# ParaGroup/WindFlow

Hardware: AMD Instinct MI355X
Metric: tuples_per_sec (higher is better)
Workload: dtype bf16; 1 GPU; model=keyed_ffat_cb_window, global_batch=16777216, win=1000, slide=100, keys_per_rank=8192, parallelism=keyed-dp1, dense_keys=True

## Files before the change

csrc/engine/bindings.cpp:

```cpp
#include <pybind11/functional.h>
#include <pybind11/numpy.h>
#include <pybind11/pybind11.h>
#include <pybind11/stl.h>

#include "engine.hpp"

namespace py = pybind11;
using namespace wfa;

static py::array col_view(DType dt, void* data, int64_t n) {
    switch (dt) {
        case DType::I64: return py::array_t<int64_t>({n}, {8}, (int64_t*)data, py::none());
        case DType::F64: return py::array_t<double>({n}, {8}, (double*)data, py::none());
        case DType::F32: return py::array_t<float>({n}, {4}, (float*)data, py::none());
        case DType::U64: return py::array_t<uint64_t>({n}, {8}, (uint64_t*)data, py::none());
        case DType::I32: return py::array_t<int32_t>({n}, {4}, (int32_t*)data, py::none());
        case DType::U16: return py::array_t<uint16_t>({n}, {2}, (uint16_t*)data, py::none());
        case DType::U8: return py::array_t<uint8_t>({n}, {1}, (uint8_t*)data, py::none());
    }
    throw std::runtime_error("bad dtype");
}

static py::dict batch_views(Batch* b, RuntimeCtx* ctx = nullptr) {
    py::dict d;
// ... 507 lines not shown
                     e.start();
                     e.wait();
                 }
             })
        .def("start",
             [](Engine& e) {
                 e.build();
                 e.start();
             })
        .def("start_gated",
             [](Engine& e) {
                 e.build();
                 {
                     py::gil_scoped_release rel;
                     e.start_gated();
                 }
             })
        .def("open_gate_and_wait",
             [](Engine& e) {
                 py::gil_scoped_release rel;
                 e.open_gate();
                 e.wait();
             })
        .def("wait",
             [](Engine& e) {
                 py::gil_scoped_release rel;
                 e.wait();
             })
        .def("abort_now", [](Engine& e) { e.abort.store(true); })
        .def("sink_sum", [](Engine& e, int op) { return e.sink_acc_i64.at(op).load(); })
        .def("sink_sum_f",
             [](Engine& e, int op) {
                 std::lock_guard<std::mutex> g(e.sink_f64_mu);
                 auto it = e.sink_acc_f64.find(op);
                 return it == e.sink_acc_f64.end() ? 0.0 : it->second;
             })
        .def("sink_count", [](Engine& e, int op) { return e.sink_tuples.at(op).load(); })
        .def("dropped", [](Engine& e) { return e.dropped_tuples.load(); })
        .def("sink_latencies",
             [](Engine& e, int op) {
                 auto it = e.sink_latencies.find(op);
                 return it == e.sink_latencies.end() ? std::vector<int64_t>{}
                                                     : it->second;
             })
        .def("stats", [](Engine& e) {
            py::list out;
            for (auto& r : e.replicas) {
                py::dict d;
                d["op"] = r->op_id;
                d["name"] = e.ops[r->op_id].name;
                d["replica"] = r->idx;
                d["inputs"] = r->stats.inputs_received;
                d["tuples_in"] = r->stats.tuples_received;
                d["outputs"] = r->stats.outputs_sent;
                d["tuples_out"] = r->stats.tuples_sent;
                d["svc_us_ewma"] = r->stats.service_time_us_ewma;
                d["start_us"] = r->stats.start_us;
                d["end_us"] = r->stats.end_us;
                d["kernels"] = r->stats.num_kernels;
                d["bytes_h2d"] = r->stats.bytes_h2d;
                d["bytes_d2h"] = r->stats.bytes_d2h;
                out.append(d);
            }
            return out;
        });

    m.def("hash_key", [](uint64_t k) { return KeyByEmitter::mix(k); });

#ifdef WFA_WITH_HIP
    m.def("debug_jit_fold_source",
          [](const std::string& kind, const std::string& spec,
             const std::vector<double>& fp, const std::vector<int64_t>& ip) {
              return debug_jit_fold_source(kind, spec, fp, ip);
          });
    m.def("debug_sort_pairs",
          [](py::array_t<uint32_t> keys, int bits) {
              auto r = debug_sort_pairs_host(keys.data(), keys.shape(0), bits);
              py::array_t<uint32_t> ks((py::ssize_t)r.first.size());
              py::array_t<uint32_t> vs((py::ssize_t)r.second.size());
              memcpy(ks.mutable_data(), r.first.data(), 4 * r.first.size());
              memcpy(vs.mutable_data(), r.second.data(), 4 * r.second.size());
              return py::make_tuple(ks, vs);
          });
    m.def("debug_ffat_stage_times",
          [](int64_t n, int64_t n_keys, int64_t win, int64_t slide, int iters,
             int vik, const std::string& fold_variant) {
              py::dict d;
              for (auto& [k, v] : debug_ffat_stage_times(n, n_keys, win, slide,
                                                         iters, vik, fold_variant))
                  d[py::str(k)] = v;
              return d;
          },
          py::arg("n"), py::arg("n_keys"), py::arg("win") = 1000,
          py::arg("slide") = 100, py::arg("iters") = 20, py::arg("vik") = 0,
          py::arg("fold_variant") = "");
    m.def("debug_tb_stage_times",
          [](int64_t n, int64_t n_keys, int iters, int mono) {
              std::map<std::string, double> m2;
              for (auto& kv : debug_tb_stage_times(n, n_keys, iters, mono))
                  m2[kv.first] = kv.second;
              return m2;
          },
          py::arg("n"), py::arg("n_keys"), py::arg("iters") = 20,
          py::arg("mono") = 1);
    m.def("debug_gram_stage_times",
          [](int64_t n, int64_t n_keys, int64_t win, int iters) {
              std::map<std::string, double> m2;
              for (auto& kv : debug_gram_stage_times(n, n_keys, win, iters))
                  m2[kv.first] = kv.second;
              return m2;
          },
          py::arg("n"), py::arg("n_keys"), py::arg("win") = 32,
          py::arg("iters") = 20);
    m.def("debug_a2a_stage_times",
          [](int64_t n, int64_t n_keys, int iters) {
              py::list out;
              for (auto& [k, v] : debug_a2a_stage_times(n, n_keys, iters))
                  out.append(py::make_tuple(k, v));
              return out;
          },
          py::arg("n"), py::arg("n_keys") = 8192, py::arg("iters") = 20);
    m.def("debug_key_slots",
          [](py::array_t<uint64_t> keys, int64_t max_keys) {
              auto r = debug_key_slots_host(keys.data(), keys.shape(0), max_keys);
              py::array_t<uint32_t> s((py::ssize_t)r.size());
              memcpy(s.mutable_data(), r.data(), 4 * r.size());
              return s;
          });
#endif

    struct StateStore {
        std::shared_ptr<void> holder;
        void* kv = nullptr;
        void* cache = nullptr;
    };
    py::class_<StateStore>(m, "StateStore")
        .def(py::init([](const std::string& path, int64_t cache_cap, bool fresh) {
                 auto s = new StateStore();
                 s->holder =
                     open_state_store(path, cache_cap, &s->kv, &s->cache, fresh);
                 return s;
             }),
             py::arg("path"), py::arg("cache_capacity") = 1 << 16,
             py::arg("fresh") = true)
        .def("erase",
             [](StateStore& s, uint64_t key) {
                 return state_kv_erase(s.kv, s.cache, key);
             })
        .def("get",
             [](StateStore& s, uint64_t key) -> py::object {
                 std::string* v = state_cache_get(s.cache, key);
                 if (!v) return py::none();
                 return py::bytes(*v);
             })
        .def("put",
             [](StateStore& s, uint64_t key, py::bytes val) {
                 state_cache_put(s.cache, key, std::string(val));
             })
        .def("flush", [](StateStore& s) { state_cache_flush(s.cache); })
        .def("__len__", [](StateStore& s) { return state_kv_size(s.kv); });
}
```

csrc/engine/engine.hpp:

```cpp
#pragma once

#include <chrono>
#include <deque>
#include <functional>
#include <thread>
#include <unordered_map>

#include "core.hpp"
#include "queue.hpp"

namespace wfa {

struct Engine;
struct Replica;

inline int64_t now_us() {
    return std::chrono::duration_cast<std::chrono::microseconds>(
               std::chrono::steady_clock::now().time_since_epoch())
        .count();
}

struct StatsRecord {
    int64_t inputs_received = 0;
    int64_t tuples_received = 0;
// ... 309 lines not shown
    std::atomic<int> gate{0};
    std::atomic<int> warmed{0};
    bool use_gate = false;
    std::unordered_map<int, std::atomic<int64_t>> sink_acc_i64;
    std::unordered_map<int, double> sink_acc_f64;
    std::mutex sink_f64_mu;
    std::unordered_map<int, std::atomic<int64_t>> sink_tuples;
    std::unordered_map<int, std::vector<int64_t>> sink_latencies;
    int64_t queue_capacity = 128;
    bool pin_threads = false;
    int dist_rank = 0;
    int dist_world = 1;
    std::string rccl_id;

    Pool* make_pool(const Schema& s, int64_t cap, bool pinned) {
        pools.push_back(std::make_unique<Pool>(s, cap, pinned));
        return pools.back().get();
    }

    void build();
    void start();
    void wait();
    void run() { build(); start(); wait(); }
    void start_gated();
    void open_gate() { gate.store(1, std::memory_order_release); }
};

std::shared_ptr<OpLogic> make_native_logic(const std::string& kind,
                                           const std::string& spec,
                                           const std::vector<double>& fparams,
                                           const std::vector<int64_t>& iparams,
                                           Engine* eng, int op_id);

struct WinRows {
    int64_t n = 0;
    const int64_t* ts = nullptr;
    uint64_t key = 0;
    int64_t gwid = 0;
    const Schema* schema = nullptr;
    std::vector<const char*> cols;
};
using WindowFn = std::function<double(const WinRows&)>;

struct JoinPairs {
    int64_t n = 0;
    const uint64_t* key = nullptr;
    const int64_t* ts_a = nullptr;
    const int64_t* ts_b = nullptr;
    const double* va = nullptr;
    const double* vb = nullptr;
};
using JoinFn =
    std::function<void(const JoinPairs&, uint8_t* keep, double* out)>;

std::shared_ptr<OpLogic> make_window_logic(const std::string& kind,
                                           const std::vector<double>& fp,
                                           const std::vector<int64_t>& ip,
                                           Engine* eng, int op_id,
                                           WindowFn userfn = nullptr,
                                           JoinFn joinfn = nullptr);

std::shared_ptr<OpLogic> make_gpu_logic(const std::string& kind, const std::string& spec,
                                        const std::vector<double>& fp,
                                        const std::vector<int64_t>& ip, Engine* eng,
                                        int op_id, int device, const Schema& os,
                                        int64_t out_batch);

std::shared_ptr<OpLogic> make_persist_logic(const std::string& kind,
                                            const std::string& spec,
                                            const std::vector<double>& fp,
                                            const std::vector<int64_t>& ip,
                                            Engine* eng, int op_id);
std::shared_ptr<void> open_state_store(const std::string& path, int64_t cache_cap,
                                       void** kv_out, void** cache_out,
                                       bool fresh = true);
std::string* state_cache_get(void* cache, uint64_t key);
void state_cache_put(void* cache, uint64_t key, const std::string& v);
void state_cache_flush(void* cache);
int64_t state_kv_size(void* kv);
bool state_kv_erase(void* kv, void* cache, uint64_t key);

std::pair<std::vector<uint32_t>, std::vector<uint32_t>> debug_sort_pairs_host(
    const uint32_t* keys, int64_t n, int bits);
std::vector<uint32_t> debug_key_slots_host(const uint64_t* keys, int64_t n,
                                           int64_t max_keys);
std::vector<std::pair<std::string, double>> debug_ffat_stage_times(
    int64_t n, int64_t n_keys, int64_t win, int64_t slide, int iters, int vik,
    const std::string& fold_variant = "");
std::vector<std::pair<std::string, double>> debug_gram_stage_times(
    int64_t n, int64_t n_keys, int64_t win, int iters);
std::vector<std::pair<std::string, double>> debug_tb_stage_times(
    int64_t n, int64_t n_keys, int iters, int mono);
std::vector<std::pair<std::string, double>> debug_a2a_stage_times(
    int64_t n, int64_t n_keys, int iters);

std::string wfa_rccl_unique_id();

std::string debug_jit_fold_source(const std::string& kind,
                                  const std::string& spec,
                                  const std::vector<double>& fp,
                                  const std::vector<int64_t>& ip);

}
```

csrc/engine/gpu_ops.cpp:

```cpp
#include <cstring>
#include <deque>
#include <map>
#include <tuple>

#include "engine.hpp"

#ifdef WFA_WITH_HIP
#include <rccl/rccl.h>

#include "../hip/wfa_kernels.h"
#include "gpu_common.hpp"

namespace wfa {

struct AuxPool {
    std::mutex mu;
    std::vector<std::pair<void*, int64_t*>> free_list;
    std::pair<void*, int64_t*> get(int device) {
        {
            std::lock_guard<std::mutex> g(mu);
            if (!free_list.empty()) {
                auto p = free_list.back();
                free_list.pop_back();
                return p;
// ... 1413 lines not shown
        hipEvent_t ev_free = ev_dest[dest_flip];
        dest_flip ^= 1;
        if (db->ready_event)
            HIPCHK(hipStreamWaitEvent(meta_stream, (hipEvent_t)db->ready_event, 0));
        HIPCHK(hipStreamWaitEvent(meta_stream, ev_free, 0));
        wfa_bucket_by_key_h(meta_stream, db->key, n, world, dest, hi);
        wfa_count_u32(meta_stream, dest, n, d_counts, world);
        HIPCHK(hipEventRecord(ev_counts, meta_stream));
        start_meta(true, wm, false);
        Meta m = sync_meta(true);
        if (m.remote_in == 0 && m.remote_out == 0 &&
            !getenv("WFA_XCHG_NO_SELFPASS")) {
            release(sb);
            int64_t out_wm = m.min_wm == WM_MAX ? cur_wm : m.min_wm;
            cur_wm = std::max(cur_wm, out_wm);
            db->watermark = out_wm;
            if (ctx.stats) ctx.stats->num_kernels += 3;
            out.emit(db);
            if (wfa_prof())
                fprintf(stderr, "[prof] xchg n=%ld self-forward meta=%ld us\n",
                        (long)n, (long)(now_us() - t1));
            return;
        }
        HIPCHK(hipStreamWaitEvent(stream, ev_counts, 0));
        uint32_t *od, *oi;
        wfa_sort_pairs2_ph(stream, dest, idx, dest_t, idx_t, nullptr, nullptr,
                           hi, n, bits, &od, &oi, nullptr, 1,
                           0);
        HIPCHK(hipEventRecord(ev_free, stream));
        size_t nc = db->cols.size();
        std::vector<void*> ptrs(2 * nc);
        for (size_t c = 0; c < nc; ++c) {
            ptrs[c] = db->cols[c];
            ptrs[nc + c] = sb->cols[c];
        }
        HIPCHK(hipMemcpyAsync(d_colptrs, ptrs.data(), 8 * 2 * nc,
                              hipMemcpyHostToDevice, stream));
        wfa_gather_rows(stream, oi, n, db->ts, sb->ts, db->key, sb->key,
                        (const void* const*)d_colptrs, (void* const*)(d_colptrs + nc),
                        d_esize, (int)nc);
        release_after_use(db);
        if (ctx.stats) ctx.stats->num_kernels += 4;
        int64_t t2 = now_us();
        round(sb, out, ctx);
        release(sb);
        if (wfa_prof())
            fprintf(stderr, "[prof] xchg n=%ld in+get=%ld us bucket=%ld us round=%ld us\n",
                    (long)n, (long)(t1 - t0), (long)(t2 - t1), (long)(now_us() - t2));
    }

    bool on_punct(int64_t, EmitCtx&, RuntimeCtx&) override { return true; }

    void on_eos(EmitCtx& out, RuntimeCtx& ctx) override {
        ensure_init();
        if (world == 1 && !getenv("WFA_XCHG_NO_SELFPASS")) return;
        for (;;) {
            start_meta(false, cur_wm, true);
            if (round(nullptr, out, ctx)) break;
        }
    }
};

std::pair<std::vector<uint32_t>, std::vector<uint32_t>> debug_sort_pairs_host(
    const uint32_t* keys, int64_t n, int bits) {
    HIPCHK(hipSetDevice(0));
    auto& A = arena(0);
    uint32_t* d_k = (uint32_t*)A.get(4 * n);
    uint32_t* d_v = (uint32_t*)A.get(4 * n);
    uint32_t* d_kt = (uint32_t*)A.get(4 * n);
    uint32_t* d_vt = (uint32_t*)A.get(4 * n);
    uint32_t* d_h = (uint32_t*)A.get(4 * wfa_sort_hist_u32(n));
    HIPCHK(hipMemcpy(d_k, keys, 4 * n, hipMemcpyHostToDevice));
    wfa_iota_u32(nullptr, d_v, n);
    uint32_t *ok, *ov;
    wfa_sort_pairs(nullptr, d_k, d_v, d_kt, d_vt, d_h, n, bits, &ok, &ov);
    std::vector<uint32_t> hk(n), hv(n);
    HIPCHK(hipMemcpy(hk.data(), ok, 4 * n, hipMemcpyDeviceToHost));
    HIPCHK(hipMemcpy(hv.data(), ov, 4 * n, hipMemcpyDeviceToHost));
    A.put(d_k, 4 * n); A.put(d_v, 4 * n); A.put(d_kt, 4 * n); A.put(d_vt, 4 * n);
    A.put(d_h, 4 * wfa_sort_hist_u32(n));
    return {std::move(hk), std::move(hv)};
}

std::vector<uint32_t> debug_key_slots_host(const uint64_t* keys, int64_t n,
                                           int64_t max_keys) {
    HIPCHK(hipSetDevice(0));
    auto& A = arena(0);
    int64_t cap = 1;
    while (cap < 2 * max_keys) cap <<= 1;
    uint64_t* d_key = (uint64_t*)A.get(8 * n);
    uint64_t* d_tab = (uint64_t*)A.get(16 * cap);
    uint32_t* d_ns = (uint32_t*)A.get(64);
    uint32_t* d_out = (uint32_t*)A.get(4 * n);
    uint64_t* d_s2k = (uint64_t*)A.get(8 * max_keys);
    HIPCHK(hipMemcpy(d_key, keys, 8 * n, hipMemcpyHostToDevice));
    wfa_fill_u64(nullptr, d_tab, ~0ULL, 2 * cap);
    wfa_fill_u32(nullptr, d_ns, 0, 1);
    wfa_key_to_slot(nullptr, d_key, n, d_tab, d_ns, cap, d_out, d_s2k);
    std::vector<uint32_t> out(n);
    HIPCHK(hipMemcpy(out.data(), d_out, 4 * n, hipMemcpyDeviceToHost));
    A.put(d_key, 8 * n); A.put(d_tab, 16 * cap);
    A.put(d_ns, 64); A.put(d_out, 4 * n); A.put(d_s2k, 8 * max_keys);
    return out;
}

std::shared_ptr<OpLogic> make_gpu_logic(const std::string& kind, const std::string& spec,
                                        const std::vector<double>& fp,
                                        const std::vector<int64_t>& ip, Engine* eng,
                                        int op_id, int device, const Schema& os,
                                        int64_t out_batch) {
    if (kind == "gpu_source")
        return std::make_shared<GpuSourceLogic>(ip[0], ip[1], ip[2], (int)ip[3],
                                                (uint64_t)ip[4], device, os);
    if (kind == "gpu_map")
        return std::make_shared<GpuMapLogic>((int)ip[0], (int)ip[1], fp[0], fp[1],
                                             device, os);
    if (kind == "gpu_filter")
        return std::make_shared<GpuFilterLogic>((int)ip[0], (int)ip[1], fp[0], fp[1],
                                                device, os, out_batch);
    if (kind == "gpu_jit_map")
        return std::make_shared<GpuJitMapLogic>(spec, (int)(ip.empty() ? 0 : ip[0]),
                                                device, os);
    if (kind == "gpu_jit_filter")
        return std::make_shared<GpuJitFilterLogic>(spec, (int)(ip.empty() ? 0 : ip[0]),
                                                   device, os, out_batch);
    if (kind == "gpu_jit_reduce" || kind == "gpu_jit_ffat" ||
        kind == "gpu_jit_stateful" || kind == "gpu_split")
        return make_gpu_jit_logic(kind, spec, fp, ip, eng, op_id, device, os,
                                  out_batch);
    if (kind == "gpu_map_keyed")
        return std::make_shared<GpuStatefulMapLogic>((int)ip[0], (int)ip[1], fp[0],
                                                     fp[1], ip[2], device, os,
                                                     out_batch);
    if (kind == "gpu_filter_keyed")
        return std::make_shared<GpuStatefulFilterLogic>((int)ip[0], (int)ip[1], fp[0],
                                                        fp[1], ip[2], device, os,
                                                        out_batch);
    if (kind == "gpu_reduce_all")
        return std::make_shared<GpuReduceAllLogic>((int)ip[0], (int)ip[1], device,
                                                   os, out_batch);
    if (kind == "gpu_reduce")
        return std::make_shared<GpuReduceLogic>((int)ip[0], (int)ip[1], ip[2], device,
                                                os, out_batch,
                                                ip.size() > 3 && ip[3] != 0);
    if (kind == "gpu_ffat") {
        auto l = std::make_shared<GpuFfatLogic>(
            (int)ip[0], (int)ip[1], ip[2], ip[3], ip[4], ip[5] != 0, device, os,
            out_batch, ip.size() > 6 && ip[6] != 0, ip.size() > 7 ? ip[7] : 0,
            ip.size() > 8 ? (int)ip[8] : 0, ip.size() > 9 && ip[9] != 0);
        l->eng_ = eng;
        return l;
    }
    if (kind == "gpu_gram") {
        auto l = std::make_shared<GpuGramLogic>(ip[0], ip[1], device, os,
                                                out_batch);
        l->ks.dense = ip.size() > 2 && ip[2] != 0;
        return l;
    }
    if (kind == "gpu_exchange")
        return std::make_shared<GpuExchangeLogic>(eng, device, os, out_batch);
    if (kind == "gpu_to_host")
        return std::make_shared<GpuToHostLogic>(device);
    if (kind == "gpu_count_sink") {
        eng->sink_acc_i64[op_id].store(0);
        eng->sink_tuples[op_id].store(0);
        return std::make_shared<GpuCountSink>(eng, op_id, device);
// ... 298 lines not shown
    float* d_cols[16];
    for (int c = 0; c < 16; ++c) {
        d_cols[c] = (float*)A.get(4 * n);
        wfa_gen_batch(s, d_ts, d_key, d_cols[c], 2, n, 0, 1000 + c, n_keys);
    }
    int64_t fires16 = (n / std::max<int64_t>(win, 1) + n_keys + 64) * 16;
    uint32_t* st_fill = (uint32_t*)A.get(4 * n_keys);
    uint32_t* st_head = (uint32_t*)A.get(4 * n_keys);
    float* st_acc = (float*)A.get(4 * n_keys * 256);
    uint32_t* nf = (uint32_t*)A.get(4 * (fires16 + 1));
    uint64_t* o_key = (uint64_t*)A.get(8 * fires16);
    int64_t* o_gwid = (int64_t*)A.get(8 * fires16);
    int64_t* o_ts = (int64_t*)A.get(8 * fires16);
    float* o_cols[16];
    for (int c = 0; c < 16; ++c) o_cols[c] = (float*)A.get(4 * fires16);
    int64_t* d_on = (int64_t*)A.get(64);
    uint32_t* d_inv = (uint32_t*)A.get(4 * n);
    float* d_staged = (float*)A.get(64 * n);
    const float** d_in = (const float**)A.get(16 * 8);
    float** d_out = (float**)A.get(16 * 8);
    HIPCHK(hipMemcpyAsync(d_in, d_cols, 16 * 8, hipMemcpyHostToDevice, s));
    HIPCHK(hipMemcpyAsync(d_out, o_cols, 16 * 8, hipMemcpyHostToDevice, s));
    HIPCHK(hipMemsetAsync(st_fill, 0, 4 * n_keys, s));
    HIPCHK(hipMemsetAsync(st_head, 0, 4 * n_keys, s));
    HIPCHK(hipMemsetAsync(st_acc, 0, 4 * n_keys * 256, s));

    constexpr int NS = 5;
    const char* names[NS] = {"group", "fire_offsets", "stage_rows", "mfma_fold",
                             "gflops"};
    hipEvent_t ev[NS];
    for (auto& e : ev) HIPCHK(hipEventCreate(&e));
    double acc[NS] = {0};
    RuntimeCtx rctx;
    for (int it = -2; it < iters; ++it) {
        HIPCHK(hipEventRecord(ev[0], s));
        wfa_key_to_slot(s, d_key, n, ks.tab, ks.d_nslots, ks.table_cap,
                        ks.slot, ks.slot_to_key);
        uint32_t *os_, *oi;
        wfa_sort_pairs2(s, ks.slot, ks.idx, ks.slot_t, ks.idx_t, nullptr,
                        nullptr, ks.hist, n, ks.bits, &os_, &oi, nullptr, 1, 0);
        ks.segs(s, os_, n, 0);
        HIPCHK(hipEventRecord(ev[1], s));
        wfa_ffat_fire_offsets(s, ks.seg_start, ks.seg_slot, ks.d_nseg, n, win,
                              1, 1, st_fill, st_head, nf, d_on, nullptr,
                              nullptr, nullptr);
        HIPCHK(hipEventRecord(ev[2], s));
        wfa_gram_prep(s, d_in, oi, n, d_inv, d_staged);
        HIPCHK(hipEventRecord(ev[3], s));
        wfa_gram_fold(s, ks.seg_start, ks.seg_slot, ks.d_nseg, n, d_in, oi,
                      d_ts, win, st_fill, st_acc, st_head, ks.slot_to_key, nf,
                      o_key, o_gwid, d_out, o_ts, fires16, d_on, d_inv,
                      d_staged);
        HIPCHK(hipEventRecord(ev[4], s));
        HIPCHK(hipStreamSynchronize(s));
        if (it >= 0)
            for (int k = 0; k < NS - 1; ++k) {
                float ms = 0;
                HIPCHK(hipEventElapsedTime(&ms, ev[k], ev[k + 1]));
                acc[k] += ms * 1000.0;
            }
    }
    for (auto& e : ev) (void)hipEventDestroy(e);
    std::vector<std::pair<std::string, double>> out;
    for (int k = 0; k < NS - 1; ++k) out.push_back({names[k], acc[k] / iters});
    double fold_us = acc[3] / iters;
    out.push_back({"gflops", fold_us > 0 ? (512.0 * n) / (fold_us * 1e3) : 0});
    return out;
}

}

#else

namespace wfa {
Batch* gpu_alloc_batch(Pool&) { throw std::runtime_error("built without HIP"); }
void gpu_free_batch(Batch*) {}
void gpu_resolve_count(Batch*) {}
Batch* gpu_clone_batch(Batch*) { throw std::runtime_error("built without HIP"); }
std::string wfa_rccl_unique_id() { throw std::runtime_error("built without HIP"); }
std::pair<std::vector<uint32_t>, std::vector<uint32_t>> debug_sort_pairs_host(
    const uint32_t*, int64_t, int) {
    throw std::runtime_error("built without HIP");
}
std::vector<uint32_t> debug_key_slots_host(const uint64_t*, int64_t, int64_t) {
    throw std::runtime_error("built without HIP");
}
std::vector<std::pair<std::string, double>> debug_ffat_stage_times(int64_t, int64_t,
                                                                   int64_t, int64_t,
                                                                   int, int,
                                                                   const std::string&) {
    throw std::runtime_error("built without HIP");
}
std::vector<std::pair<std::string, double>> debug_a2a_stage_times(int64_t, int64_t,
                                                                  int) {
    throw std::runtime_error("built without HIP");
}
std::vector<std::pair<std::string, double>> debug_gram_stage_times(int64_t,
                                                                   int64_t,
                                                                   int64_t,
                                                                   int) {
    throw std::runtime_error("built without HIP");
}
std::vector<std::pair<std::string, double>> debug_tb_stage_times(int64_t,
                                                                 int64_t, int,
                                                                 int) {
    throw std::runtime_error("built without HIP");
}
std::shared_ptr<OpLogic> make_gpu_logic(const std::string&, const std::string&,
                                        const std::vector<double>&,
                                        const std::vector<int64_t>&, Engine*, int, int,
                                        const Schema&, int64_t) {
    throw std::runtime_error("built without HIP");
}
}

#endif
```

csrc/hip/sortwin.hip:

```cpp
#include <hip/hip_runtime.h>

#include <cstdio>
#include <cstdlib>

#include "wfa_kernels.h"

static int wfa_sort_dbg() {
    static int v = -1;
    if (v < 0) v = getenv("WFA_DEBUG_SYNC") ? 1 : 0;
    return v;
}
static void sdbg(hipStream_t st, const char* what, int pass) {
    if (!wfa_sort_dbg()) return;
    hipError_t e = hipStreamSynchronize(st);
    hipError_t e2 = hipGetLastError();
    fprintf(stderr, "[sortdbg] p%d %s sync=%s last=%s\n", pass, what,
            hipGetErrorString(e), hipGetErrorString(e2));
    fflush(stderr);
}

#define WFA_THREADS 256
#define WFA_MAX_BLOCKS 2048
#define RS_IPT 8
#define RS_PER_BLOCK (WFA_THREADS * RS_IPT)
// ... 602 lines not shown
    __shared__ uint32_t sk[RS8_PER_BLOCK];
    __shared__ uint32_t sv[RS8_PER_BLOCK];
    __shared__ uint32_t sv2[CARRY2 ? RS8_PER_BLOCK : 1];
    __shared__ uint8_t sd[RS8_PER_BLOCK];
    const int wave = threadIdx.x >> 6, lane = threadIdx.x & 63;
    const uint64_t lt = ((uint64_t)1 << lane) - 1;
    for (int d = threadIdx.x; d < 256; d += blockDim.x) {
        gbase[d] = hist[(int64_t)d * nblocks + blockIdx.x] + dbase[d];
        for (int w = 0; w < WFA_THREADS / 64; ++w) waveCnt[w][d] = 0;
    }
    __syncthreads();
    int64_t blockStart = (int64_t)blockIdx.x * RS8_PER_BLOCK;
    int64_t waveBase = blockStart + wave * RS8_PER_WAVE;
    uint32_t mk[RS8_IPT], mv[RS8_IPT], mv2[RS8_IPT], mr[RS8_IPT];
    int nit = 0;
#pragma unroll
    for (int j = 0; j < RS8_IPT; ++j) {
        int64_t i = waveBase + j * 64 + lane;
        bool valid = i < n;
        uint32_t k = valid ? keys[i] : 0;
        uint32_t v = valid ? (vals ? vals[i] : (uint32_t)i) : 0;
        uint32_t d = (k >> shift) & 255;
        uint64_t mask = __ballot(valid);
#pragma unroll
        for (int bit = 0; bit < 8; ++bit) {
            uint64_t b = __ballot((d >> bit) & 1);
            mask &= ((d >> bit) & 1) ? b : ~b;
        }
        if (valid) {
            uint32_t pre = waveCnt[wave][d];
            uint32_t rank = pre + (uint32_t)__popcll(mask & lt);
            mk[j] = k;
            mv[j] = v;
            if (CARRY2) mv2[j] = vals2[i];
            mr[j] = (d << 24) | (rank & 0xFFFFFF);
            if ((mask & lt) == 0) waveCnt[wave][d] = pre + (uint32_t)__popcll(mask);
            nit = j + 1;
        }
    }
    __syncthreads();
    __shared__ uint32_t blockCnt[256];
    for (int d = threadIdx.x; d < 256; d += blockDim.x) {
        uint32_t run = 0;
        for (int w = 0; w < WFA_THREADS / 64; ++w) {
            wavePre[w][d] = run;
            run += waveCnt[w][d];
        }
        blockCnt[d] = run;
    }
    __syncthreads();
    if (threadIdx.x < 256) {
        __shared__ uint32_t tot[256];
        uint32_t c = blockCnt[threadIdx.x];
        tot[threadIdx.x] = c;
        __syncthreads();
        for (int off = 1; off < 256; off <<= 1) {
            uint32_t t = (threadIdx.x >= off) ? tot[threadIdx.x - off] : 0;
            __syncthreads();
            tot[threadIdx.x] += t;
            __syncthreads();
        }
        localBase[threadIdx.x] = tot[threadIdx.x] - c;
    }
    __syncthreads();
    for (int j = 0; j < nit; ++j) {
        uint32_t d = mr[j] >> 24;
        uint32_t lpos = localBase[d] + wavePre[wave][d] + (mr[j] & 0xFFFFFF);
        sk[lpos] = mk[j];
        sv[lpos] = mv[j];
        if (CARRY2) sv2[lpos] = mv2[j];
        sd[lpos] = (uint8_t)d;
    }
    __syncthreads();
    const int nblk_items = (int)min((int64_t)RS8_PER_BLOCK, n - blockStart);
    for (int p = threadIdx.x; p < nblk_items; p += blockDim.x) {
        uint32_t d = sd[p];
        uint32_t g = gbase[d] + (uint32_t)p - localBase[d];
        keys_out[g] = sk[p];
        vals_out[g] = sv[p];
        if (CARRY2) vals2_out[g] = sv2[p];
    }
}

static void sort_pairs2_impl(wfa_stream_t s, uint32_t* slot, uint32_t* idx,
                             uint32_t* slot_tmp, uint32_t* idx_tmp,
                             uint32_t* val2, uint32_t* val2_tmp,
                             uint32_t* hist, int64_t n, int bits,
                             uint32_t** out_slot, uint32_t** out_idx,
                             uint32_t** out_val2, int implicit_iota,
                             int base_shift, int skip_hist0) {
    hipStream_t st = (hipStream_t)s;
    uint32_t *ka = slot, *va = idx, *kb = slot_tmp, *vb = idx_tmp;
    uint32_t *wa = val2, *wb = val2_tmp;
    bool first = true;
    if (bits > 4) {
        int64_t nb = wfa_sort8_nblocks(n);
        uint32_t* dt = hist + 256 * nb;
        uint32_t* dbase = dt + 256;
        int passes = (bits + 7) / 8;
        for (int p = 0; p < passes; ++p) {
            int shift = base_shift + 8 * p;
            if (!(p == 0 && skip_hist0)) {
                hipLaunchKernelGGL(k_rs8_hist, dim3(nb), dim3(WFA_THREADS), 0, st,
                                   ka, n, shift, hist, nb);
            }
            sdbg(st, "hist", p);
            hipLaunchKernelGGL(k_rs8_scan, dim3(256), dim3(256), 0, st, hist, nb, dt);
            sdbg(st, "scan", p);
            hipLaunchKernelGGL(k_rs8_dbase, dim3(1), dim3(256), 0, st, dt, dbase);
            sdbg(st, "dbase", p);
            uint32_t* va_eff = (first && implicit_iota) ? nullptr : va;
            if (val2)
                hipLaunchKernelGGL(k_rs8_scatter_lds<true>, dim3(nb),
                                   dim3(WFA_THREADS), 0, st, ka, va_eff, n, shift,
                                   hist, nb, dbase, kb, vb, wa, wb);
            else
                hipLaunchKernelGGL(k_rs8_scatter_lds<false>, dim3(nb),
                                   dim3(WFA_THREADS), 0, st, ka, va_eff, n, shift,
                                   hist, nb, dbase, kb, vb, wa, wb);
            sdbg(st, "scatter", p);
            first = false;
            uint32_t* t;
            t = ka; ka = kb; kb = t;
            t = va; va = vb; vb = t;
            t = wa; wa = wb; wb = t;
        }
        *out_slot = ka;
        *out_idx = va;
        if (out_val2) *out_val2 = wa;
        return;
    }
    int64_t nblocks = wfa_sort_nblocks(n);
    uint32_t* dt = hist + 16 * nblocks;
    int passes = (bits + 3) / 4;
    (void)base_shift;
    for (int p = 0; p < passes; ++p) {
        int shift = 4 * p;
        hipLaunchKernelGGL(k_rs_hist, dim3(nblocks), dim3(WFA_THREADS), 0, st, ka, n,
                           shift, hist, nblocks);
        hipLaunchKernelGGL(k_rs_scan16, dim3(16), dim3(256), 0, st, hist, nblocks, dt);
        hipLaunchKernelGGL(k_rs_scatter, dim3(nblocks), dim3(WFA_THREADS), 0, st, ka,
                           (first && implicit_iota) ? nullptr : va, n, shift, hist,
                           nblocks, dt, kb, vb, wa, wb);
        first = false;
        uint32_t* t;
        t = ka; ka = kb; kb = t;
        t = va; va = vb; vb = t;
        t = wa; wa = wb; wb = t;
    }
    *out_slot = ka;
    *out_idx = va;
    if (out_val2) *out_val2 = wa;
}

extern "C" void wfa_sort_pairs2(wfa_stream_t s, uint32_t* slot, uint32_t* idx,
                                uint32_t* slot_tmp, uint32_t* idx_tmp,
                                uint32_t* val2, uint32_t* val2_tmp,
                                uint32_t* hist, int64_t n, int bits,
                                uint32_t** out_slot, uint32_t** out_idx,
                                uint32_t** out_val2, int implicit_iota,
                                int base_shift) {
    sort_pairs2_impl(s, slot, idx, slot_tmp, idx_tmp, val2, val2_tmp, hist, n,
                     bits, out_slot, out_idx, out_val2, implicit_iota,
                     base_shift, 0);
}

extern "C" void wfa_sort_pairs2_ph(wfa_stream_t s, uint32_t* slot, uint32_t* idx,
                                   uint32_t* slot_tmp, uint32_t* idx_tmp,
                                   uint32_t* val2, uint32_t* val2_tmp,
                                   uint32_t* hist, int64_t n, int bits,
                                   uint32_t** out_slot, uint32_t** out_idx,
                                   uint32_t** out_val2, int implicit_iota,
                                   int base_shift) {
    sort_pairs2_impl(s, slot, idx, slot_tmp, idx_tmp, val2, val2_tmp, hist, n,
                     bits, out_slot, out_idx, out_val2, implicit_iota,
                     base_shift, bits > 4 ? 1 : 0);
}

extern "C" void wfa_sort_pairs(wfa_stream_t s, uint32_t* slot, uint32_t* idx,
                               uint32_t* slot_tmp, uint32_t* idx_tmp, uint32_t* hist,
                               int64_t n, int bits, uint32_t** out_slot,
                               uint32_t** out_idx) {
    wfa_sort_pairs2(s, slot, idx, slot_tmp, idx_tmp, nullptr, nullptr, hist, n,
                    bits, out_slot, out_idx, nullptr, 0, 0);
}

__global__ void k_seg_count(const uint32_t* slot, int64_t n, uint32_t* blk_cnt,
                            int shr) {
    int64_t base = (int64_t)blockIdx.x * RS_PER_BLOCK + (int64_t)threadIdx.x * RS_IPT;
    uint32_t c = 0;
#pragma unroll
    for (int j = 0; j < RS_IPT; ++j) {
        int64_t i = base + j;
        if (i < n) c += (i == 0) || ((slot[i] >> shr) != (slot[i - 1] >> shr));
    }
    __shared__ uint32_t red[WFA_THREADS / 64];
    for (int off = 32; off; off >>= 1) c += __shfl_down(c, off, 64);
    if ((threadIdx.x & 63) == 0) red[threadIdx.x >> 6] = c;
    __syncthreads();
    if (threadIdx.x == 0) {
        uint32_t t = 0;
        for (int w = 0; w < WFA_THREADS / 64; ++w) t += red[w];
        blk_cnt[blockIdx.x] = t;
    }
}

__global__ void k_seg_scatter(const uint32_t* slot, int64_t n, const uint32_t* blk_off,
                              uint32_t* seg_start, uint32_t* seg_slot, int shr) {
    int64_t base = (int64_t)blockIdx.x * RS_PER_BLOCK + (int64_t)threadIdx.x * RS_IPT;
    uint32_t c = 0;
#pragma unroll
    for (int j = 0; j < RS_IPT; ++j) {
        int64_t i = base + j;
        if (i < n) c += (i == 0) || ((slot[i] >> shr) != (slot[i - 1] >> shr));
    }
    __shared__ uint32_t tc[WFA_THREADS];
    tc[threadIdx.x] = c;
    __syncthreads();
    for (int off = 1; off < WFA_THREADS; off <<= 1) {
        uint32_t t = (threadIdx.x >= off) ? tc[threadIdx.x - off] : 0;
        __syncthreads();
        tc[threadIdx.x] += t;
        __syncthreads();
    }
    uint32_t w = blk_off[blockIdx.x] + tc[threadIdx.x] - c;
    for (int j = 0; j < RS_IPT; ++j) {
        int64_t i = base + j;
        if (i >= n) continue;
        if ((i == 0) || ((slot[i] >> shr) != (slot[i - 1] >> shr))) {
            seg_start[w] = (uint32_t)i;
            seg_slot[w] = slot[i] >> shr;
            ++w;
        }
    }
}

__global__ void k_nseg_total(const uint32_t* slot_sorted, int64_t n,
                             const uint32_t* scan_tmp, int64_t nb, int64_t* d_nseg,
                             int shr) {
    if (blockIdx.x == 0 && threadIdx.x < 64) {
        int64_t base = (nb - 1) * (int64_t)RS_PER_BLOCK;
        uint32_t c = 0;
        for (int64_t i = base + threadIdx.x; i < n; i += 64)
            c += (i == 0) || ((slot_sorted[i] >> shr) != (slot_sorted[i - 1] >> shr));
        for (int off = 32; off; off >>= 1) c += __shfl_down(c, off, 64);
        if (threadIdx.x == 0) *d_nseg = (int64_t)scan_tmp[nb - 1] + c;
    }
}

__global__ void k_seg_by_slot(const uint32_t* slot, int64_t n, uint32_t* by_slot,
                              int shr) {
    for (int64_t i = blockIdx.x * (int64_t)blockDim.x + threadIdx.x; i < n;
         i += gridDim.x * (int64_t)blockDim.x) {
        uint32_t sl = slot[i] >> shr;
        if (i == 0 || (slot[i - 1] >> shr) != sl) by_slot[sl] = (uint32_t)i;
    }
}

#define SEGC_BLOCKS 32
// ... 2030 lines not shown
```

csrc/hip/wfa_kernels.h:

```cpp
#pragma once
#include <cstdint>

typedef void* wfa_stream_t;

extern "C" {

void wfa_gen_batch(wfa_stream_t s, int64_t* ts, uint64_t* key, void* val, int vdt,
                   int64_t n, int64_t start, uint64_t seed, uint64_t n_keys);

void wfa_map_apply(wfa_stream_t s, int spec, void* col, int dt, int64_t n,
                   double a, double b);

void wfa_filter_flags(wfa_stream_t s, int spec, const void* col, int dt, int64_t n,
                      double a, double b, uint32_t* flags);

void wfa_compact(wfa_stream_t s, int64_t n, const uint32_t* flags,
                 uint32_t* scan_tmp,
                 const int64_t* ts_in, int64_t* ts_out,
                 const uint64_t* key_in, uint64_t* key_out,
                 const void* const* cols_in, void* const* cols_out,
                 const int* col_esize, int n_cols, int64_t* d_count);

void wfa_key_to_slot_v(wfa_stream_t s, const uint64_t* key, int64_t n,
                       uint64_t* table_packed, uint32_t* n_slots,
                       int64_t table_cap, uint32_t* slot_out,
                       uint64_t* slot_to_key, const uint16_t* val);
void wfa_key_to_slot(wfa_stream_t s, const uint64_t* key, int64_t n,
                     uint64_t* table_packed, uint32_t* n_slots,
                     int64_t table_cap, uint32_t* slot_out,
                     uint64_t* slot_to_key);
void wfa_key_dense(wfa_stream_t s, const uint64_t* key, int64_t n,
                   int64_t max_keys, uint32_t* slot_out, uint32_t* n_slots,
                   uint32_t* overflow, const uint16_t* val);
void wfa_key_to_slot_h(wfa_stream_t s, const uint64_t* key, int64_t n,
                       uint64_t* table_packed, uint32_t* n_slots,
                       int64_t table_cap, uint32_t* slot_out,
                       uint64_t* slot_to_key, const uint16_t* val,
                       uint32_t* hist, int shift);
void wfa_key_dense_h(wfa_stream_t s, const uint64_t* key, int64_t n,
                     int64_t max_keys, uint32_t* slot_out, uint32_t* n_slots,
                     uint32_t* overflow, const uint16_t* val, uint32_t* hist,
                     int shift);
void wfa_iota_u64(wfa_stream_t s, uint64_t* p, int64_t n);
void wfa_bucket_by_key_h(wfa_stream_t s, const uint64_t* key, int64_t n,
                         int world, uint32_t* dest, uint32_t* hist);

void wfa_sort_pairs(wfa_stream_t s, uint32_t* slot, uint32_t* idx,
                    uint32_t* slot_tmp, uint32_t* idx_tmp, uint32_t* hist,
                    int64_t n, int bits,
                    uint32_t** out_slot, uint32_t** out_idx);
void wfa_sort_pairs2(wfa_stream_t s, uint32_t* slot, uint32_t* idx,
                     uint32_t* slot_tmp, uint32_t* idx_tmp,
                     uint32_t* val2, uint32_t* val2_tmp, uint32_t* hist,
                     int64_t n, int bits, uint32_t** out_slot,
                     uint32_t** out_idx, uint32_t** out_val2,
                     int implicit_iota, int base_shift);
void wfa_sort_pairs2_ph(wfa_stream_t s, uint32_t* slot, uint32_t* idx,
                        uint32_t* slot_tmp, uint32_t* idx_tmp,
                        uint32_t* val2, uint32_t* val2_tmp, uint32_t* hist,
                        int64_t n, int bits, uint32_t** out_slot,
                        uint32_t** out_idx, uint32_t** out_val2,
                        int implicit_iota, int base_shift);
int64_t wfa_sort_nblocks(int64_t n);
int64_t wfa_sort_hist_u32(int64_t cap);

void wfa_gather(wfa_stream_t s, const uint32_t* idx, int64_t n,
                const void* v_in, void* v_out, int esize,
                const int64_t* ts_in, int64_t* ts_out);

void wfa_segments(wfa_stream_t s, const uint32_t* slot_sorted, int64_t n,
                  uint32_t* scan_tmp, uint32_t* seg_start, uint32_t* seg_slot,
                  int64_t* d_nseg, int shr);
void wfa_segments_dense(wfa_stream_t s, const uint32_t* slot_sorted, int64_t n,
                        uint32_t* by_slot, int64_t max_slots,
                        uint32_t* scratch32, uint32_t* seg_start,
                        uint32_t* seg_slot, int64_t* d_nseg, int shr);

void wfa_segment_reduce(wfa_stream_t s, const uint32_t* seg_start,
                        const uint32_t* seg_slot, const int64_t* d_nseg, int64_t n,
                        const void* v_orig, const uint32_t* idx_sorted,
                        const int64_t* ts_orig, int vdt,
                        int comb, const uint64_t* slot_to_key,
                        uint64_t* out_key, void* out_val, int64_t* out_ts,
                        int64_t* d_out_n);
void wfa_segment_reduce_wave(
    wfa_stream_t s, const uint32_t* seg_start, const uint32_t* seg_slot,
    const int64_t* d_nseg, int64_t n, const void* v_orig, int vdt,
    const uint32_t* idx_sorted, const int64_t* ts_orig, int comb, int ts_last,
    const uint64_t* slot_to_key, uint64_t* out_key, void* out_val,
    int64_t* out_ts, int64_t* d_out_n);

void wfa_ffat_fire_offsets(wfa_stream_t s, const uint32_t* seg_start,
                           const uint32_t* seg_slot, const int64_t* d_nseg,
                           int64_t n, int64_t pane_len, int64_t P, int64_t S,
                           const uint32_t* st_fill, const uint32_t* st_head,
                           uint32_t* nf, int64_t* d_out_n,
                           const uint32_t* idx_sorted, const int64_t* ts_orig,
                           int64_t* st_last);

void wfa_ffat_fire_offsets_pw(
    wfa_stream_t s, const uint32_t* seg_start, const uint32_t* seg_slot,
    const int64_t* d_nseg, int64_t n, int64_t pane_len, int64_t P, int64_t S,
    const uint32_t* st_fill, const uint32_t* st_head, uint32_t* nf,
    int64_t* d_out_n, const uint32_t* idx_sorted, const int64_t* ts_orig,
    int64_t* st_last, uint32_t* pane_base, int64_t* d_total_panes);
void wfa_ffat_cb_fold_pw(
    wfa_stream_t s, const uint32_t* seg_start, const uint32_t* seg_slot,
    const int64_t* d_nseg, const int64_t* d_total_panes, int64_t n,
    const void* v_f32, int vdt, const uint32_t* idx_sorted,
    const int64_t* ts_orig, int64_t pane_len, int64_t P, int64_t S, int comb,
    int ring_log2, int64_t* st_count, uint32_t* st_fill, float* st_acc,
    float* st_acc_new, float* ring, uint32_t* st_head, float* st_wsum,
    const uint64_t* slot_to_key, const uint32_t* fire_base,
    const uint32_t* pane_base, float* temp, uint64_t* out_key, float* out_val,
    int64_t* out_ts, int64_t out_cap);

enum {
    WFA_CB_FOLD_WAVE = 0,
    WFA_CB_FOLD_TILE = 1,
    WFA_CB_FOLD_TILE512 = 2,
    WFA_CB_FOLD_TILE2048 = 3,
};
void wfa_ffat_cb_fold(wfa_stream_t s, const uint32_t* seg_start,
                      const uint32_t* seg_slot, const int64_t* d_nseg, int64_t n,
                      const void* v_f32, int vdt, const uint32_t* idx_sorted,
                      const int64_t* ts_orig,
                      int64_t pane_len, int64_t P, int64_t S, int comb,
                      int ring_log2,
                      int64_t* st_count, uint32_t* st_fill, float* st_acc,
                      float* ring, uint32_t* st_head, float* st_wsum,
                      const uint64_t* slot_to_key, const uint32_t* fire_base,
                      uint64_t* out_key, float* out_val, int64_t* out_ts,
                      int64_t out_cap, int variant);

void wfa_ffat_cb_fold_fused(
    wfa_stream_t s, const uint32_t* seg_start, const uint32_t* seg_slot,
    const int64_t* d_nseg, int64_t n, const void* v_f32, int vdt,
    const uint32_t* idx_sorted, const int64_t* ts_orig, int64_t pane_len,
    int64_t P, int64_t S, int comb, int ring_log2, int64_t* st_count,
    uint32_t* st_fill, float* st_acc, float* ring, uint32_t* st_head,
    float* st_wsum, const uint64_t* slot_to_key, const uint32_t* fire_base,
    uint64_t* out_key, float* out_val, int64_t* out_ts, int64_t out_cap);

void wfa_gram_prep(wfa_stream_t s, const float* const* colp,
                   const uint32_t* idx_sorted, int64_t n,
// ... 118 lines not shown
```

Measured before the change: 31.66 billion tuples/s.

## Add ballot-based radix scatter kernel as default, dropping dbase launch

Adds a new onepass-style radix-sort scatter kernel that ranks digits within each wave using ballot bit-matching and per-wave LDS counters. It computes digit bases inside the block, so the separate single-block dbase kernel is no longer launched. The launch bounds are set for higher occupancy. It becomes the default for sort_pairs2, with the old LDS scatter kept behind an env var, and a debug binding is added for testing variants. Risk: the extra ballots and LDS staging passes could cost more than the occupancy gain.

```diff
diff --git a/csrc/engine/bindings.cpp b/csrc/engine/bindings.cpp
--- a/csrc/engine/bindings.cpp
+++ b/csrc/engine/bindings.cpp
@@ -613,6 +613,36 @@
               memcpy(vs.mutable_data(), r.second.data(), 4 * r.second.size());
               return py::make_tuple(ks, vs);
           });
+    m.def("debug_sort_pairs2",
+          [](py::array_t<uint32_t, py::array::c_style | py::array::forcecast> keys,
+             int bits, int base_shift, bool implicit_iota, bool prehist,
+             py::object vals2, const std::string& variant) {
+              const int64_t n = keys.shape(0);
+              py::array_t<uint32_t, py::array::c_style | py::array::forcecast> v2;
+              const uint32_t* v2p = nullptr;
+              if (!vals2.is_none()) {
+                  v2 = vals2.cast<py::array_t<uint32_t, py::array::c_style |
+                                                            py::array::forcecast>>();
+                  if (v2.ndim() != 1 || v2.shape(0) != n)
+                      throw std::runtime_error("debug_sort_pairs2: vals2 length");
+                  v2p = v2.data();
+              }
+              auto r = debug_sort_pairs2_host(keys.data(), n, bits, base_shift,
+                                              implicit_iota, prehist, v2p, variant);
+              py::array_t<uint32_t> ks((py::ssize_t)n), vs((py::ssize_t)n);
+              memcpy(ks.mutable_data(), r.keys.data(), 4 * n);
+              memcpy(vs.mutable_data(), r.idx.data(), 4 * n);
+              py::object w = py::none();
+              if (v2p) {
+                  py::array_t<uint32_t> ws((py::ssize_t)n);
+                  memcpy(ws.mutable_data(), r.vals2.data(), 4 * n);
+                  w = ws;
+              }
+              return py::make_tuple(ks, vs, w);
+          },
+          py::arg("keys"), py::arg("bits"), py::arg("base_shift") = 0,
+          py::arg("implicit_iota") = true, py::arg("prehist") = false,
+          py::arg("vals2") = py::none(), py::arg("variant") = "");
     m.def("debug_ffat_stage_times",
           [](int64_t n, int64_t n_keys, int64_t win, int64_t slide, int iters,
              int vik, const std::string& fold_variant) {
diff --git a/csrc/engine/engine.hpp b/csrc/engine/engine.hpp
--- a/csrc/engine/engine.hpp
+++ b/csrc/engine/engine.hpp
@@ -415,6 +415,13 @@
 
 std::pair<std::vector<uint32_t>, std::vector<uint32_t>> debug_sort_pairs_host(
     const uint32_t* keys, int64_t n, int bits);
+struct DebugSort2 {
+    std::vector<uint32_t> keys, idx, vals2;
+};
+DebugSort2 debug_sort_pairs2_host(const uint32_t* keys, int64_t n, int bits,
+                                  int base_shift, bool implicit_iota,
+                                  bool prehist, const uint32_t* vals2,
+                                  const std::string& variant);
 std::vector<uint32_t> debug_key_slots_host(const uint64_t* keys, int64_t n,
                                            int64_t max_keys);
 std::vector<std::pair<std::string, double>> debug_ffat_stage_times(
diff --git a/csrc/engine/gpu_ops.cpp b/csrc/engine/gpu_ops.cpp
--- a/csrc/engine/gpu_ops.cpp
+++ b/csrc/engine/gpu_ops.cpp
@@ -1519,6 +1519,74 @@
     return {std::move(hk), std::move(hv)};
 }
 
+DebugSort2 debug_sort_pairs2_host(const uint32_t* keys, int64_t n, int bits,
+                                  int base_shift, bool implicit_iota,
+                                  bool prehist, const uint32_t* vals2,
+                                  const std::string& variant) {
+    int var;
+    if (variant.empty()) var = 0;
+    else if (variant == "occ") var = 1;
+    else if (variant == "lds") var = 2;
+    else throw std::runtime_error("debug_sort_pairs2: unknown variant '" + variant + "'");
+    if (n < 1 || bits < 1 || base_shift < 0 || base_shift + bits > 32)
+        throw std::runtime_error("debug_sort_pairs2: bad n / bits / base_shift");
+    if (prehist && base_shift != 0 && base_shift != 16)
+        throw std::runtime_error("debug_sort_pairs2: prehist needs base_shift 0 or 16");
+    HIPCHK(hipSetDevice(0));
+    auto& A = arena(0);
+    const size_t hb = 4 * wfa_sort_hist_u32(n);
+    uint32_t* d_k = (uint32_t*)A.get(4 * n);
+    uint32_t* d_v = (uint32_t*)A.get(4 * n);
+    uint32_t* d_kt = (uint32_t*)A.get(4 * n);
+    uint32_t* d_vt = (uint32_t*)A.get(4 * n);
+    uint32_t* d_w = vals2 ? (uint32_t*)A.get(4 * n) : nullptr;
+    uint32_t* d_wt = vals2 ? (uint32_t*)A.get(4 * n) : nullptr;
+    uint32_t* d_h = (uint32_t*)A.get(hb);
+    if (vals2) HIPCHK(hipMemcpy(d_w, vals2, 4 * n, hipMemcpyHostToDevice));
+    if (!implicit_iota) wfa_iota_u32(nullptr, d_v, n);
+    if (prehist) {
+        std::vector<uint64_t> hk(n);
+        std::vector<uint16_t> hv(n);
+        for (int64_t i = 0; i < n; ++i) {
+            hk[i] = keys[i] >> base_shift;
+            hv[i] = (uint16_t)(keys[i] & 0xFFFF);
+        }
+        uint64_t* d_key = (uint64_t*)A.get(8 * n);
+        uint16_t* d_val = (uint16_t*)A.get(2 * n);
+        uint32_t* d_ns = (uint32_t*)A.get(64);
+        HIPCHK(hipMemcpy(d_key, hk.data(), 8 * n, hipMemcpyHostToDevice));
+        HIPCHK(hipMemcpy(d_val, hv.data(), 2 * n, hipMemcpyHostToDevice));
+        wfa_fill_u32(nullptr, d_ns, 0, 2);
+        wfa_key_dense_h(nullptr, d_key, n, (int64_t)1 << bits, d_k, d_ns, d_ns + 1,
+                        base_shift ? d_val : nullptr, d_h, base_shift);
+        HIPCHK(hipStreamSynchronize(nullptr));
+        A.put(d_key, 8 * n); A.put(d_val, 2 * n); A.put(d_ns, 64);
+    } else {
+        HIPCHK(hipMemcpy(d_k, keys, 4 * n, hipMemcpyHostToDevice));
+    }
+    uint32_t *ok, *ov, *ow = nullptr;
+    if (prehist && var == 0)
+        wfa_sort_pairs2_ph(nullptr, d_k, d_v, d_kt, d_vt, d_w, d_wt, d_h, n, bits,
+                           &ok, &ov, &ow, implicit_iota ? 1 : 0, base_shift);
+    else
+        wfa_sort_pairs2_ex(nullptr, d_k, d_v, d_kt, d_vt, d_w, d_wt, d_h, n, bits,
+                           &ok, &ov, &ow, implicit_iota ? 1 : 0, base_shift,
+                           prehist ? 1 : 0, var, nullptr, nullptr);
+    DebugSort2 r;
+    r.keys.resize(n);
+    r.idx.resize(n);
+    HIPCHK(hipMemcpy(r.keys.data(), ok, 4 * n, hipMemcpyDeviceToHost));
+    HIPCHK(hipMemcpy(r.idx.data(), ov, 4 * n, hipMemcpyDeviceToHost));
+    if (vals2) {
+        r.vals2.resize(n);
+        HIPCHK(hipMemcpy(r.vals2.data(), ow, 4 * n, hipMemcpyDeviceToHost));
+    }
+    A.put(d_k, 4 * n); A.put(d_v, 4 * n); A.put(d_kt, 4 * n); A.put(d_vt, 4 * n);
+    if (vals2) { A.put(d_w, 4 * n); A.put(d_wt, 4 * n); }
+    A.put(d_h, hb);
+    return r;
+}
+
 std::vector<uint32_t> debug_key_slots_host(const uint64_t* keys, int64_t n,
                                            int64_t max_keys) {
     HIPCHK(hipSetDevice(0));
@@ -1983,6 +2051,10 @@
     const uint32_t*, int64_t, int) {
     throw std::runtime_error("built without HIP");
 }
+DebugSort2 debug_sort_pairs2_host(const uint32_t*, int64_t, int, int, bool, bool,
+                                  const uint32_t*, const std::string&) {
+    throw std::runtime_error("built without HIP");
+}
 std::vector<uint32_t> debug_key_slots_host(const uint64_t*, int64_t, int64_t) {
     throw std::runtime_error("built without HIP");
 }
diff --git a/csrc/hip/sortwin.hip b/csrc/hip/sortwin.hip
--- a/csrc/hip/sortwin.hip
+++ b/csrc/hip/sortwin.hip
@@ -708,13 +708,179 @@
     }
 }
 
+__device__ __forceinline__ uint32_t rs8_wave_incl_scan(uint32_t v, int lane) {
+#pragma unroll
+    for (int o = 1; o < 64; o <<= 1) {
+        uint32_t t = (uint32_t)__shfl_up((int)v, o, 64);
+        if (lane >= o) v += t;
+    }
+    return v;
+}
+
+template <bool CARRY2>
+__global__ void __launch_bounds__(WFA_THREADS, CARRY2 ? 5 : 6)
+k_rs8_scatter_occ(const uint32_t* keys, const uint32_t* vals, int64_t n,
+                  int shift, const uint32_t* hist, int64_t nblocks,
+                  const uint32_t* dt, uint32_t* keys_out, uint32_t* vals_out,
+                  const uint32_t* vals2, uint32_t* vals2_out) {
+    static_assert(WFA_THREADS == 256, "one thread per digit");
+    static_assert(RS8_PER_BLOCK <= 65536, "staged position packs in 16 bits");
+    __shared__ uint32_t stage[RS8_PER_BLOCK];
+    __shared__ uint32_t cnt[WFA_THREADS / 64][256];
+    __shared__ uint32_t gd[256];
+    __shared__ uint32_t wtot[2][WFA_THREADS / 64];
+    const int tid = threadIdx.x;
+    const int wave = tid >> 6, lane = tid & 63;
+    const uint64_t lt = ((uint64_t)1 << lane) - 1;
+    const int64_t blockStart = (int64_t)blockIdx.x * RS8_PER_BLOCK;
+    const int nblk_items = (int)min((int64_t)RS8_PER_BLOCK, n - blockStart);
+    const int li0 = wave * RS8_PER_WAVE + lane;
+    const uint32_t* kblk = keys + blockStart;
+    const uint32_t hbase = hist[(int64_t)tid * nblocks + blockIdx.x];
+    const uint32_t dtv = dt[tid];
+#pragma unroll
+    for (int w = 0; w < WFA_THREADS / 64; ++w) cnt[w][tid] = 0;
+    uint32_t mk[RS8_IPT];
+#pragma unroll
+    for (int j = 0; j < RS8_IPT; ++j) {
+        int li = li0 + j * 64;
+        mk[j] = (li < nblk_items) ? kblk[li] : 0;
+    }
+    __syncthreads();
+    uint32_t mr[RS8_IPT];
+#pragma unroll
+    for (int j = 0; j < RS8_IPT; ++j) {
+        bool valid = li0 + j * 64 < nblk_items;
+        uint32_t d = (mk[j] >> shift) & 255;
+#ifdef RS8_OCC_MATCH_SELECT
+        uint64_t mask = __ballot(valid);
+#pragma unroll
+        for (int bit = 0; bit < 8; ++bit) {
+            uint64_t b = __ballot((d >> bit) & 1);
+            mask &= ((d >> bit) & 1) ? b : ~b;
+        }
+#else
+        uint32_t dlo = 0, dhi = 0;
+#pragma unroll
+        for (int bit = 0; bit < 8; ++bit) {
+            int32_t s = (int32_t)(d << (31 - bit)) >> 31;
+            uint64_t b = __ballot(s != 0);
+            dlo |= (uint32_t)b ^ (uint32_t)s;
+            dhi |= (uint32_t)(b >> 32) ^ (uint32_t)s;
+        }
+        uint64_t mask = __ballot(valid) & ~(((uint64_t)dhi << 32) | dlo);
+#endif
+        mr[j] = 0;
+        if (valid) {
+            uint32_t pre = cnt[wave][d];
+            mr[j] = pre + (uint32_t)__popcll(mask & lt);
+            if ((mask & lt) == 0) cnt[wave][d] = pre + (uint32_t)__popcll(mask);
+        }
+    }
+    __syncthreads();
+    {
+        uint32_t c0 = cnt[0][tid], c1 = cnt[1][tid], c2 = cnt[2][tid],
+                 c3 = cnt[3][tid];
+        uint32_t c = c0 + c1 + c2 + c3;
+        uint32_t ic = rs8_wave_incl_scan(c, lane);
+        uint32_t id = rs8_wave_incl_scan(dtv, lane);
+        if (lane == 63) {
+            wtot[0][wave] = ic;
+            wtot[1][wave] = id;
+        }
+        __syncthreads();
+        uint32_t oc = 0, od = 0;
+#pragma unroll
+        for (int w = 0; w < WFA_THREADS / 64 - 1; ++w)
+            if (w < wave) {
+                oc += wtot[0][w];
+                od += wtot[1][w];
+            }
+        uint32_t lb = ic - c + oc;
+        uint32_t db = id - dtv + od;
+        cnt[0][tid] = lb;
+        cnt[1][tid] = lb + c0;
+        cnt[2][tid] = lb + c0 + c1;
+        cnt[3][tid] = lb + c0 + c1 + c2;
+        gd[tid] = hbase + db - lb;
+    }
+    __syncthreads();
+#pragma unroll
+    for (int j = 0; j < RS8_IPT; ++j) {
+        if (li0 + j * 64 < nblk_items) {
+            uint32_t d = (mk[j] >> shift) & 255;
+            mr[j] += cnt[wave][d];
+            stage[mr[j]] = mk[j];
+        }
+    }
+    uint32_t mv[RS8_IPT];
+#pragma unroll
+    for (int j = 0; j < RS8_IPT; ++j) {
+        int li = li0 + j * 64;
+        mv[j] = (li < nblk_items)
+                    ? (vals ? vals[blockStart + li] : (uint32_t)blockStart + (uint32_t)li)
+                    : 0;
+    }
+    __syncthreads();
+#pragma unroll
+    for (int j = 0; j < RS8_IPT; ++j) {
+        int p = tid + j * WFA_THREADS;
+        if (p < nblk_items) {
+            uint32_t k = stage[p];
+            uint32_t d = (k >> shift) & 255;
+            keys_out[gd[d] + (uint32_t)p] = k;
+            mr[j] |= d << 16;
+        }
+    }
+    __syncthreads();
+#pragma unroll
+    for (int j = 0; j < RS8_IPT; ++j)
+        if (li0 + j * 64 < nblk_items) stage[mr[j] & 0xFFFF] = mv[j];
+    if (CARRY2) {
+#pragma unroll
+        for (int j = 0; j < RS8_IPT; ++j) {
+            int li = li0 + j * 64;
+            mv[j] = (li < nblk_items) ? vals2[blockStart + li] : 0;
+        }
+    }
+    __syncthreads();
+#pragma unroll
+    for (int j = 0; j < RS8_IPT; ++j) {
+        int p = tid + j * WFA_THREADS;
+        if (p < nblk_items) vals_out[gd[mr[j] >> 16] + (uint32_t)p] = stage[p];
+    }
+    if (CARRY2) {
+        __syncthreads();
+#pragma unroll
+        for (int j = 0; j < RS8_IPT; ++j)
+            if (li0 + j * 64 < nblk_items) stage[mr[j] & 0xFFFF] = mv[j];
+        __syncthreads();
+#pragma unroll
+        for (int j = 0; j < RS8_IPT; ++j) {
+            int p = tid + j * WFA_THREADS;
+            if (p < nblk_items) vals2_out[gd[mr[j] >> 16] + (uint32_t)p] = stage[p];
+        }
+    }
+}
+
+static int wfa_rs8_env_lds() {
+    static int v = -1;
+    if (v < 0) {
+        const char* e = getenv("WFA_RS8_SCATTER");
+        v = (e && e[0] == 'l' && e[1] == 'd' && e[2] == 's' && e[3] == 0) ? 1 : 0;
+    }
+    return v;
+}
+
 static void sort_pairs2_impl(wfa_stream_t s, uint32_t* slot, uint32_t* idx,
                              uint32_t* slot_tmp, uint32_t* idx_tmp,
                              uint32_t* val2, uint32_t* val2_tmp,
                              uint32_t* hist, int64_t n, int bits,
                              uint32_t** out_slot, uint32_t** out_idx,
                              uint32_t** out_val2, int implicit_iota,
-                             int base_shift, int skip_hist0) {
+                             int base_shift, int skip_hist0, int variant = 0,
+                             wfa_sort_probe_t probe = nullptr,
+                             void* probe_ctx = nullptr) {
     hipStream_t st = (hipStream_t)s;
     uint32_t *ka = slot, *va = idx, *kb = slot_tmp, *vb = idx_tmp;
     uint32_t *wa = val2, *wb = val2_tmp;
@@ -724,26 +890,42 @@
         uint32_t* dt = hist + 256 * nb;
         uint32_t* dbase = dt + 256;
         int passes = (bits + 7) / 8;
+        const bool lds = variant ? variant == 2 : wfa_rs8_env_lds() != 0;
         for (int p = 0; p < passes; ++p) {
             int shift = base_shift + 8 * p;
             if (!(p == 0 && skip_hist0)) {
                 hipLaunchKernelGGL(k_rs8_hist, dim3(nb), dim3(WFA_THREADS), 0, st,
                                    ka, n, shift, hist, nb);
+                if (probe) probe(probe_ctx, "hist", p);
             }
             sdbg(st, "hist", p);
             hipLaunchKernelGGL(k_rs8_scan, dim3(256), dim3(256), 0, st, hist, nb, dt);
+            if (probe) probe(probe_ctx, "scan", p);
             sdbg(st, "scan", p);
-            hipLaunchKernelGGL(k_rs8_dbase, dim3(1), dim3(256), 0, st, dt, dbase);
-            sdbg(st, "dbase", p);
             uint32_t* va_eff = (first && implicit_iota) ? nullptr : va;
-            if (val2)
-                hipLaunchKernelGGL(k_rs8_scatter_lds<true>, dim3(nb),
-                                   dim3(WFA_THREADS), 0, st, ka, va_eff, n, shift,
-                                   hist, nb, dbase, kb, vb, wa, wb);
-            else
-                hipLaunchKernelGGL(k_rs8_scatter_lds<false>, dim3(nb),
-                                   dim3(WFA_THREADS), 0, st, ka, va_eff, n, shift,
-                                   hist, nb, dbase, kb, vb, wa, wb);
+            if (lds) {
+                hipLaunchKernelGGL(k_rs8_dbase, dim3(1), dim3(256), 0, st, dt, dbase);
+                if (probe) probe(probe_ctx, "dbase", p);
+                sdbg(st, "dbase", p);
+                if (val2)
+                    hipLaunchKernelGGL(k_rs8_scatter_lds<true>, dim3(nb),
+                                       dim3(WFA_THREADS), 0, st, ka, va_eff, n, shift,
+                                       hist, nb, dbase, kb, vb, wa, wb);
+                else
+                    hipLaunchKernelGGL(k_rs8_scatter_lds<false>, dim3(nb),
+                                       dim3(WFA_THREADS), 0, st, ka, va_eff, n, shift,
+                                       hist, nb, dbase, kb, vb, wa, wb);
+            } else {
+                if (val2)
+                    hipLaunchKernelGGL(k_rs8_scatter_occ<true>, dim3(nb),
+                                       dim3(WFA_THREADS), 0, st, ka, va_eff, n, shift,
+                                       hist, nb, dt, kb, vb, wa, wb);
+                else
+                    hipLaunchKernelGGL(k_rs8_scatter_occ<false>, dim3(nb),
+                                       dim3(WFA_THREADS), 0, st, ka, va_eff, n, shift,
+                                       hist, nb, dt, kb, vb, wa, wb);
+            }
+            if (probe) probe(probe_ctx, "scatter", p);
             sdbg(st, "scatter", p);
             first = false;
             uint32_t* t;
@@ -801,6 +983,20 @@
     sort_pairs2_impl(s, slot, idx, slot_tmp, idx_tmp, val2, val2_tmp, hist, n,
                      bits, out_slot, out_idx, out_val2, implicit_iota,
                      base_shift, bits > 4 ? 1 : 0);
+}
+
+extern "C" void wfa_sort_pairs2_ex(wfa_stream_t s, uint32_t* slot, uint32_t* idx,
+                                   uint32_t* slot_tmp, uint32_t* idx_tmp,
+                                   uint32_t* val2, uint32_t* val2_tmp,
+                                   uint32_t* hist, int64_t n, int bits,
+                                   uint32_t** out_slot, uint32_t** out_idx,
+                                   uint32_t** out_val2, int implicit_iota,
+                                   int base_shift, int skip_hist0, int variant,
+                                   wfa_sort_probe_t probe, void* probe_ctx) {
+    sort_pairs2_impl(s, slot, idx, slot_tmp, idx_tmp, val2, val2_tmp, hist, n,
+                     bits, out_slot, out_idx, out_val2, implicit_iota,
+                     base_shift, (skip_hist0 && bits > 4) ? 1 : 0, variant, probe,
+                     probe_ctx);
 }
 
 extern "C" void wfa_sort_pairs(wfa_stream_t s, uint32_t* slot, uint32_t* idx,
diff --git a/csrc/hip/wfa_kernels.h b/csrc/hip/wfa_kernels.h
--- a/csrc/hip/wfa_kernels.h
+++ b/csrc/hip/wfa_kernels.h
@@ -61,6 +61,14 @@
                         int64_t n, int bits, uint32_t** out_slot,
                         uint32_t** out_idx, uint32_t** out_val2,
                         int implicit_iota, int base_shift);
+typedef void (*wfa_sort_probe_t)(void* ctx, const char* kernel, int pass);
+void wfa_sort_pairs2_ex(wfa_stream_t s, uint32_t* slot, uint32_t* idx,
+                        uint32_t* slot_tmp, uint32_t* idx_tmp,
+                        uint32_t* val2, uint32_t* val2_tmp, uint32_t* hist,
+                        int64_t n, int bits, uint32_t** out_slot,
+                        uint32_t** out_idx, uint32_t** out_val2,
+                        int implicit_iota, int base_shift, int skip_hist0,
+                        int variant, wfa_sort_probe_t probe, void* probe_ctx);
 int64_t wfa_sort_nblocks(int64_t n);
 int64_t wfa_sort_hist_u32(int64_t cap);
 
```

Measured after the change: 38.61 billion tuples/s, median of 6. 21.9% higher.
